# John-Jumper/Upside-MD

Measured on AMD Instinct MI355X. Metric: MD steps/sec (force evals/sec) per 300-res protein, higher is better.
Workload: dtype f32; 1 GPU; syn300_10A: 300-res synthetic protein, full side-chain BP, 10 A pair list (BASELINE.json configs[2]); 4096 independent replicas per GPU, T=0.8, dt=0.009, Langevin thermostat every round; replicas_per_gpu=4096, n_atom=900, settle_steps=100

## Files before the change

upside-md_amd/csrc/igraph_device.h:

```cpp
#pragma once
#include "device_math.h"
#include "../../include/upside_hip_kernels.h"
#include <hip/amd_detail/amd_hip_unsafe_atomics.h>

#include "env_switch.h"

struct BX { int bx, gx, by, gy; };
#define BX_REAL (BX{(int)blockIdx.x, (int)gridDim.x, (int)blockIdx.y, (int)gridDim.y})

namespace up {

__device__ __forceinline__ void bspline_basis(float y, float b[4], float d[4]) {
    const float y2 = y * y, omy = 1.f - y, omy2 = omy * omy;
    const float s = 1.f / 6.f;
    b[0] = omy2 * (omy * s);
    b[1] = fmaf(fmaf(0.5f, y, -1.f), y2, 2.f / 3.f);
    b[2] = fmaf(fmaf(fmaf(-0.5f, y, 0.5f), y, 0.5f), y, s);
    b[3] = y2 * (y * s);
    d[0] = -0.5f * omy2;
    d[1] = y * fmaf(1.5f, y, -2.f);
    d[2] = fmaf(fmaf(-1.5f, y, 1.f), y, 0.5f);
    d[3] = 0.5f * y2;
}
template <typename P>
// ... 234 lines not shown
    if (PG_LANES == 16) v += dpp_mov<UP_DPP_ROW_MIRROR>(v);
    if (PG_LANES >= 8) v += dpp_mov<UP_DPP_HALF_MIRROR>(v);
    v += dpp_mov<UP_DPP_XOR2>(v);
    v += dpp_mov<UP_DPP_XOR1>(v);
    return v;
}

template <int IT> struct list_word { typedef unsigned short type; };
template <> struct list_word<UPK_IT_ROTAMER> { typedef int type; };
static inline bool list_words_match(const upk_igraph_t* G) { return (G->word16 != 0) == (G->itype != UPK_IT_ROTAMER); }
__device__ __forceinline__ int list_word_at(const int* lists, size_t idx, int word16) {
    return word16 ? (int)((const unsigned short*)lists)[idx] : lists[idx];
}

__device__ __forceinline__ void stage_ranges(int* lds_range, unsigned short* lds_ord, const int* __restrict__ hcnt, const int* __restrict__ hlo,
                                             const unsigned short* __restrict__ ord, int n_rows) {
    for (int t = threadIdx.x; t < n_rows; t += blockDim.x) {
        lds_range[t] = (hlo ? hlo[t] : 0) | (hcnt[t] << 16);
        lds_ord[t] = ord[t];
    }
}
#define PG_WALK_LDS_WORDS(n_rows) ((n_rows) + ((n_rows) + 1) / 2)

template <typename Op, int LANES = PG_LANES, typename W = int>
__device__ __forceinline__ void group_batch_loop(Op& op, int n_rows, const unsigned short* ord, const int* range,
                                                 const W* __restrict__ hit, int cap, int* counter, int batch_first, int batch_step) {
    const int lane = threadIdx.x & 63, gl = lane & (LANES - 1), g = lane / LANES;
    const int n_batch = (n_rows + (UP_WAVE / LANES) - 1) / (UP_WAVE / LANES);
    auto claim = [&]() { int v = 0; if (lane == 0) v = atomicAdd(counter, 1); return __builtin_amdgcn_readfirstlane(v); };
    struct Batch { int row, n_mine; const W* hrow; int w[PG_CHUNK]; bool valid; };
    auto fetch = [&](int i, Batch& B) -> bool {
        const int b = batch_first + i * batch_step;
        if (b >= n_batch) return false;
        const int ri = b * (UP_WAVE / LANES) + g;
// ... 32 lines not shown
}

static inline void pair_geometry(int n_system, int n_rows, int lanes_per_row, int rows_per_full_wg, int& wgs_per_system, int& threads) {
    static const int wgs_env = env_int("UPSIDE_HIP_IG_WGS", 256);
    const int target = wgs_env < 1 ? 256 : wgs_env;
    int bps = (target + n_system - 1) / n_system;
    const int max_bps = (n_rows + rows_per_full_wg - 1) / rows_per_full_wg;
    if (bps > max_bps) bps = max_bps;
    if (bps < 1) bps = 1;
    const int rows_per_wg = (n_rows + bps - 1) / bps;
    int t = ((rows_per_wg * lanes_per_row + 63) / 64) * 64;
    threads = t < 256 ? 256 : (t > 1024 ? 1024 : t);
    wgs_per_system = bps;
}

__device__ __forceinline__ float fast_rcp(float x) { return __builtin_amdgcn_rcpf(x); }

}
```

upside-md_amd/csrc/kernels_pair.hip:

```cpp
#include "igraph_device.h"
#include "pair2_device.h"
#include <cstring>

using namespace up;
typedef unsigned short PW;

#define ST(L) ((hipStream_t)(L)->stream)
#ifndef UPK_LAUNCH_STATUS_DEFINED
#define UPK_LAUNCH_STATUS_DEFINED
static inline int launch_status() { return (int)hipGetLastError(); }
#endif
#define C_SENS(c, s) ((c).sens + (size_t)(s) * (c).n_elem * (c).stride)

struct PairArgs {
    float* out; long out_sys_stride; int out_stride, out_comp, out_row0, out_row0_2;
    float* own_grad;
    int sens_mode; const float* sens1; const float* sens2; long sens_sys_stride; int sens_stride;
    int tab_floats;
    int atomic_sens;
};

template <int IT, int ROW_SIDE, bool GRAD, bool POLY>
__device__ __forceinline__ float pair_functor(const upk_igraph_t& G, const QuadShape& Q, const float* tab, int t1, int t2,
                                              const float* x1, const float* x2, float* d) {
// ... 137 lines not shown
        if (SIDES == 3) __syncthreads();
        if (threadIdx.x == 0) *L.counter = 0;
        stage_ranges(L.range, L.ord, G.hcnt2 + (size_t)s * G.n2, nullptr, G.ord2 + (size_t)s * G.n2, G.n2);
        __syncthreads();
        RowOp<IT, 2, MODE, POLY, LANES> op(G, L, A, s);
        group_batch_loop<RowOp<IT, 2, MODE, POLY, LANES>, LANES>(op, G.n2, L.ord, L.range, (const PW*)G.hit2 + (size_t)s * G.n2 * G.cap2, G.cap2, L.counter, B.bx, B.gx);
    }
}
template <int IT, int SIDES, int MODE, bool POLY>
__global__ void __launch_bounds__(1024) PG_KERNEL_ATTR k_pair_rows(upk_igraph_t G, PairArgs A)  {
    extern __shared__ __attribute__((aligned(16))) float lds_dyn_[];
    d_pair_rows<IT, SIDES, MODE, POLY>(G, A, BX_REAL, lds_dyn_);
}

template <int DO, typename Get>
__device__ __forceinline__ void flush_other_side(float* __restrict__ osens, const int* __restrict__ oloc, int stride, int n_other, Get get) {
    for (int i = threadIdx.x; i < n_other; i += blockDim.x) {
        float add[8];
#pragma unroll
        for (int c = 0; c < 8; ++c) add[c] = c < DO ? get(c, i) : 0.f;
        float4* row = (float4*)(osens + (size_t)oloc[i] * stride);
        float4 r0 = row[0];
        r0.x += add[0]; r0.y += add[1]; r0.z += add[2]; r0.w += add[3];
        if (DO > 4) { float4 r1 = row[1]; r1.x += add[4]; r1.y += add[5]; r1.z += add[6]; r1.w += add[7]; row[1] = r1; }
        row[0] = r0;
    }
}
template <int IT, int RS, bool POLY>
struct BackwardOp {
    static constexpr int DR = RS == 1 ? PairDims<IT>::d1 : PairDims<IT>::d2;
    static constexpr int DO = RS == 1 ? PairDims<IT>::d2 : PairDims<IT>::d1;
    const upk_igraph_t& G; const QuadShape Q; const PairLds& L; unsigned long long* oacc;
// ... 120 lines not shown
        load_row8_planes(xa, RS == 1 ? L.c2 : L.c1, (RS == 1 ? G.n2 : G.n1) + 1, jA); load_row8_planes(xb, RS == 1 ? L.c2 : L.c1, (RS == 1 ? G.n2 : G.n1) + 1, jB);
        v2 xo[6];
#pragma unroll
        for (int c = 0; c < 6; ++c) xo[c] = mk2(xa[c], xb[c]);
        const int toA = __float_as_int(xa[7]), toB = __float_as_int(xb[7]);
        const v2 v = RS == 1 ? coverage_pair2<false, POLY>(G, Q, L.tab, tr, tr, toA, toB, xr, hbr, xo, nullptr, nullptr)
                             : coverage_pair2<false, POLY>(G, Q, L.tab, toA, toB, tr, tr, xo, mk2(xa[6], xb[6]), xr, nullptr, nullptr);
        acc += mk2(liveA ? v.x : 0.f, liveB ? v.y : 0.f);
    }
    __device__ __forceinline__ void flush(int row) {
        const float t = group_sum4(acc.x + acc.y);
        if ((threadIdx.x & (P2_LANES - 1)) != 0) return;
        A.out[(size_t)s * A.out_sys_stride + (size_t)((RS == 1 ? A.out_row0 : A.out_row0_2) + row) * A.out_stride + A.out_comp] = t;
    }
};
template <int RS, bool POLY>
__device__ __forceinline__ void d_cov_rows2(const upk_igraph_t& G, const PairArgs& A, const BX B, float* lds) {
        const int s = B.by;
    const PairLds L = pair2_lds(lds, G, A.tab_floats);
    stage_table(L.tab, POLY ? G.param_poly : G.param, A.tab_floats);
    const int row_len = POLY ? G.n_poly : G.n_param;
    stage_rows_planes(L.c1, G.node1, s, G.loc1, G.n1, G.dim1, G.type1, nullptr, nullptr, 0, 0.f, __int_as_float(0), G.n_type2 * row_len);
    stage_rows_planes(L.c2, G.node2, s, G.loc2, G.n2, G.dim2, G.type2, nullptr, nullptr, 0, 0.f, __int_as_float(0), row_len);
    if (threadIdx.x == 0) *L.counter = 0;
    const int n_rows = RS == 1 ? G.n1 : G.n2, cap = RS == 1 ? G.cap1 : G.cap2;
    stage_ranges(L.range, L.ord, (RS == 1 ? G.hcnt1 : G.hcnt2) + (size_t)s * n_rows, nullptr, (RS == 1 ? G.ord1 : G.ord2) + (size_t)s * n_rows, n_rows);
    __syncthreads();
    CovRowOp2<RS, POLY> op(G, L, A, s);
    group2_batch_loop(op, n_rows, L.ord, L.range, (const PW*)(RS == 1 ? G.hit1 : G.hit2) + (size_t)s * n_rows * cap, cap, L.counter, B.bx, B.gx, RS == 1 ? G.n2 : G.n1);
}
template <int RS, bool POLY>
__global__ void __launch_bounds__(1024) PG_KERNEL_ATTR k_cov_rows2(upk_igraph_t G, PairArgs A)  {
    extern __shared__ __attribute__((aligned(16))) float lds_dyn_[];
    d_cov_rows2<RS, POLY>(G, A, BX_REAL, lds_dyn_);
}

template <int RS, bool POLY>
struct CovBackwardOp2 {
    static constexpr int DR = RS == 1 ? 7 : 6, DO = RS == 1 ? 6 : 7;
    const upk_igraph_t& G; const QuadShape Q; const PairLds& L; unsigned long long* oacc;
    const bool row_has, oth_has;
    v2 xr[6], hbr, acc[DR]; float sr; int tr;
    float* row_sens; const int* row_loc; int row_stride;
    __device__ __forceinline__ CovBackwardOp2(const upk_igraph_t& G_, const PairLds& L_, unsigned long long* oacc_, int sens_mode, int s)
        : G(G_), Q(quad_shape(G_)), L(L_), oacc(oacc_), row_has(sens_mode == 3 || sens_mode == RS), oth_has(sens_mode == 3 || sens_mode == 3 - RS) {
        const upk_coord_t& node = RS == 1 ? G.node1 : G.node2;
        row_sens = node.sens + (size_t)s * node.n_elem * node.stride; row_loc = RS == 1 ? G.loc1 : G.loc2; row_stride = node.stride;
    }
    const float* site_sens = nullptr;
    __device__ __forceinline__ void begin(int row) {
// ... 34 lines not shown
#pragma unroll
            for (int c = 0; c < DO; ++c) lds_add_fixed22_scaled(oacc + c * n_o + jB, od[c].y);
        }
    }
    __device__ __forceinline__ void flush(int row) {
        float t[DR];
#pragma unroll
        for (int c = 0; c < DR; ++c) t[c] = group_sum4(acc[c].x + acc[c].y);
        if ((threadIdx.x & (P2_LANES - 1)) != 0) return;
        float* o = row_sens + (size_t)row_loc[row] * row_stride;
#pragma unroll
        for (int c = 0; c < DR; ++c) o[c] += t[c];
    }
};
template <int RS, bool POLY>
__device__ __forceinline__ void d_cov_backward2(const upk_igraph_t& G, const PairArgs& A, const BX B, float* lds) {
        constexpr int DO = CovBackwardOp2<RS, POLY>::DO;
    const int s = B.by;
    const int n_rows = RS == 1 ? G.n1 : G.n2, n_other = RS == 1 ? G.n2 : G.n1;
    const PairLds L = pair2_lds(lds, G, A.tab_floats);
    unsigned long long* oacc = (unsigned long long*)lds + (((size_t)((float*)(L.counter + 1) - lds) + 1) >> 1);
    float* site_sens = (float*)(oacc + (size_t)n_other * DO);
    const float* S1 = A.sens1 ? A.sens1 + (size_t)s * A.sens_sys_stride : nullptr;
    const float* S2 = A.sens2 ? A.sens2 + (size_t)s * A.sens_sys_stride : nullptr;
    stage_table(L.tab, POLY ? G.param_poly : G.param, A.tab_floats);
    const int row_len = POLY ? G.n_poly : G.n_param;
    stage_rows_planes(L.c1, G.node1, s, G.loc1, G.n1, G.dim1, G.type1, nullptr, nullptr, 0, 0.f, __int_as_float(0), G.n_type2 * row_len);
    stage_rows_planes(L.c2, G.node2, s, G.loc2, G.n2, G.dim2, G.type2, nullptr, S2, A.sens_stride, 0.f, __int_as_float(0), row_len);
    if (S1) for (int t = threadIdx.x; t < G.n1; t += blockDim.x) site_sens[t] = S1[(size_t)t * A.sens_stride];
    for (int t = threadIdx.x; t < n_other * DO; t += blockDim.x) oacc[t] = 0ull;
    if (threadIdx.x == 0) *L.counter = 0;
    stage_ranges(L.range, L.ord, (RS == 1 ? G.hcnt1 : G.hcnt2) + (size_t)s * n_rows, nullptr, (RS == 1 ? G.ord1 : G.ord2) + (size_t)s * n_rows, n_rows);
    __syncthreads();
    {
        CovBackwardOp2<RS, POLY> op(G, L, oacc, A.sens_mode, s);
        op.site_sens = site_sens;
        const int cap = RS == 1 ? G.cap1 : G.cap2;
        group2_batch_loop(op, n_rows, L.ord, L.range, (const PW*)(RS == 1 ? G.hit1 : G.hit2) + (size_t)s * n_rows * cap, cap, L.counter, B.bx, B.gx, n_other);
    }
    __syncthreads();
    const upk_coord_t& onode = RS == 1 ? G.node2 : G.node1;
    const int* oloc = RS == 1 ? G.loc2 : G.loc1;
    float* osens = C_SENS(onode, s);
    unsigned long long* gacc = G.gacc ? G.gacc + (size_t)s * n_other * 8 : nullptr;
    const bool alone = B.gx == 1;
    if (alone && (onode.stride & 3) == 0) { flush_other_side<DO>(osens, oloc, onode.stride, n_other, [&](int c, int i) { return from_fixed22(oacc[c * n_other + i]); }); return; }
    for (int t = threadIdx.x; t < n_other * DO; t += blockDim.x) {
        const int i = t / DO, c = t - i * DO;
        const unsigned long long a = oacc[c * n_other + i];
        if (!a) continue;
        if (alone) osens[(size_t)oloc[i] * onode.stride + c] += from_fixed22(a);
        else atomicAdd(gacc + i * 8 + c, a);
    }
}
template <int RS, bool POLY>
__global__ void __launch_bounds__(1024) PG_KERNEL_ATTR k_cov_backward2(upk_igraph_t G, PairArgs A)  {
    extern __shared__ __attribute__((aligned(16))) float lds_dyn_[];
    d_cov_backward2<RS, POLY>(G, A, BX_REAL, lds_dyn_);
}

__device__ __forceinline__ void d_pair_backward_finish(const upk_igraph_t& G, int other_side, double unit, const BX B, float* lds_unused) {
    const int s = B.by;
    const int n_other = other_side == 1 ? G.n1 : G.n2, dim = other_side == 1 ? G.dim1 : G.dim2;
    const upk_coord_t& onode = other_side == 1 ? G.node1 : G.node2;
    const int* oloc = other_side == 1 ? G.loc1 : G.loc2;
    float* osens = C_SENS(onode, s);
    unsigned long long* gacc = G.gacc + (size_t)s * n_other * 8;
    for (int t = B.bx * blockDim.x + threadIdx.x; t < n_other * 8; t += B.gx * blockDim.x) {
        const int i = t >> 3, c = t & 7;
        if (c >= dim) continue;
        const unsigned long long a = gacc[t];
        if (a) { osens[(size_t)oloc[i] * onode.stride + c] += (float)((double)(long long)a * unit); gacc[t] = 0ull; }
    }
}
// ... 13 lines not shown
    if (mode == 0) hipLaunchKernelGGL((k_pair_rows<IT, SIDES, 0, POLY>), grid, block, lds, ST(L), *G, A);
    else if (mode == 1) hipLaunchKernelGGL((k_pair_rows<IT, SIDES, 1, POLY>), grid, block, lds, ST(L), *G, A);
    else hipLaunchKernelGGL((k_pair_rows<IT, SIDES, 2, POLY>), grid, block, lds, ST(L), *G, A);
}
template <int IT, bool POLY = false>
static void rows_launch_sides(const upk_launch_t* L, const upk_igraph_t* G, int side, int mode, dim3 grid, dim3 block, size_t lds, const PairArgs& A) {
    if (side == 1) rows_launch<IT, 1, POLY>(L, G, mode, grid, block, lds, A);
    else if (side == 2) rows_launch<IT, 2, POLY>(L, G, mode, grid, block, lds, A);
    else rows_launch<IT, 3, POLY>(L, G, mode, grid, block, lds, A);
}
static int pair_table_choice(const upk_igraph_t* G, size_t extra, int& tab_floats, size_t& lds) {
    static const bool no_poly = env_int("UPSIDE_HIP_IG_POLY", 1) == 0;
    if (!no_poly && pair_lds_bytes(G, true, tab_floats, lds) && lds + extra <= 158 * 1024) return 2;
    if (pair_lds_bytes(G, false, tab_floats, lds) && lds + extra <= 158 * 1024) return 1;
    return 0;
}

extern "C" int upk_igraph_passes_staged(const upk_launch_t* L, const upk_igraph_t* G, int row_side) {
    UPK_FLUSH(L);
    (void)L;
    if (row_side != 1 && row_side != 2) return 0;
    const int n_other = row_side == 1 ? G->n2 : G->n1;
    int tab_floats; size_t lds;
    if (!pair_table_choice(G, 0, tab_floats, lds)) return 0;
    return pair_table_choice(G, 8 + (size_t)n_other * 8 * sizeof(unsigned long long), tab_floats, lds) ? 1 : 0;
}

extern "C" int upk_igraph_rows(const upk_launch_t* L, const upk_igraph_t* G, int side, int mode, float* out, long out_sys_stride,
                               int out_stride, int out_comp, int out_row0, int out_row0_2, float* own_grad, int sens_mode,
                               const float* sens1, const float* sens2, long sens_sys_stride, int sens_stride) {
// ... 10 lines not shown
    if (!table) {
        UPK_FLUSH(L);
        int r = 0;
        for (int sd = 1; sd <= 2 && !r; ++sd) {
            if (!(side & sd)) continue;
            const int row0 = sd == 1 ? A.out_row0 : A.out_row0_2;
            if (mode == 2) r = upk_igraph_grad(L, G, sd, sens_mode, sens1, sens2, sens_sys_stride, sens_stride);
            else r = upk_igraph_rowsum(L, G, sd, out, out_sys_stride, out_stride, out_comp, row0, mode == 1 ? own_grad : nullptr);
        }
        return r;
    }
    const int n_rows = side == 1 ? G->n1 : (side == 2 ? G->n2 : (G->n1 > G->n2 ? G->n1 : G->n2));
    int bps, threads;
    if (G->itype == UPK_IT_HBOND_COVERAGE && mode == 0 && side != 3 && pair2_enabled() && lds + 64 <= 158 * 1024) {
        pair_geometry(L->n_system, n_rows, P2_LANES, 256, bps, threads);
        if (side == 2 && batch_add(L, table == 2 ? BK_COV_ROWS2_POLY : BK_COV_ROWS2, bps, L->n_system, lds + 64, G, sizeof(*G), &A, sizeof(A))) return 0;
        UPK_FLUSH(L);
        const dim3 grid2(bps, L->n_system), block2(threads);
        if (side == 1) { if (table == 2) hipLaunchKernelGGL((k_cov_rows2<1, true>), grid2, block2, lds + 64, ST(L), *G, A); else hipLaunchKernelGGL((k_cov_rows2<1, false>), grid2, block2, lds + 64, ST(L), *G, A); }
        else { if (table == 2) hipLaunchKernelGGL((k_cov_rows2<2, true>), grid2, block2, lds + 64, ST(L), *G, A); else hipLaunchKernelGGL((k_cov_rows2<2, false>), grid2, block2, lds + 64, ST(L), *G, A); }
        return launch_status();
    }
    pair_geometry(L->n_system, n_rows, PG_LANES, 128, bps, threads);
    if (G->itype == UPK_IT_PROTEIN_HBOND && bps == 1) {
        threads = 256;
    }
    {
        const int bk = (G->itype == UPK_IT_PROTEIN_HBOND && side == 3 && mode == 0) ? BK_ROWS_HB_FWD : (G->itype == UPK_IT_PROTEIN_HBOND && side == 3 && mode == 2) ? BK_ROWS_HB_BWD
                     : (G->itype == UPK_IT_ENVIRONMENT && side == 1 && mode == 0) ? BK_ROWS_ENV_FWD : 0;
        if (bk && batch_add(L, bk, bps, L->n_system, lds, G, sizeof(*G), &A, sizeof(A))) return 0;
// ... 37 lines not shown
    if (!table) {
        UPK_FLUSH(L);
        int r = upk_igraph_grad(L, G, 1, sens_mode, sens1, sens2, sens_sys_stride, sens_stride);
        if (!r) r = upk_igraph_grad(L, G, 2, sens_mode, sens1, sens2, sens_sys_stride, sens_stride);
        return r;
    }
    int bps, threads;
    if (G->itype == UPK_IT_HBOND_COVERAGE && pair2_enabled()) {
        const size_t extra = 64 + (size_t)G->n1 * sizeof(float);
        size_t lds2; int tf;
        const int table2 = pair_table_choice(G, acc_bytes + extra, tf, lds2);
        if (table2) {
            A.tab_floats = tf; lds2 += acc_bytes + extra;
            pair_geometry(L->n_system, n_rows, P2_LANES, 256, bps, threads);
            if (!G->gacc) bps = 1;
            if (row_side == 2 && batch_add(L, table2 == 2 ? BK_COV_BWD2_POLY : BK_COV_BWD2, bps, L->n_system, lds2, G, sizeof(*G), &A, sizeof(A))) {
                if (bps > 1 && !batch_add(L, BK_BWD_FINISH, (n_other * 8 + 1023) / 1024, L->n_system, 0, G, sizeof(*G), nullptr, 0, 3 - row_side, 0, 1.0 / (double)(1 << P2_FIX_BITS)))
                    return finish_alone(L, G, n_other, 3 - row_side, 1.0 / (double)(1 << P2_FIX_BITS));
                return 0;
            }
            UPK_FLUSH(L);
            const dim3 grid2(bps, L->n_system), block2(threads);
            if (row_side == 1) { if (table2 == 2) hipLaunchKernelGGL((k_cov_backward2<1, true>), grid2, block2, lds2, ST(L), *G, A); else hipLaunchKernelGGL((k_cov_backward2<1, false>), grid2, block2, lds2, ST(L), *G, A); }
            else { if (table2 == 2) hipLaunchKernelGGL((k_cov_backward2<2, true>), grid2, block2, lds2, ST(L), *G, A); else hipLaunchKernelGGL((k_cov_backward2<2, false>), grid2, block2, lds2, ST(L), *G, A); }
            if (bps > 1) hipLaunchKernelGGL(k_pair_backward_finish, dim3((n_other * 8 + 255) / 256, L->n_system), dim3(256), 0, ST(L), *G, 3 - row_side, 1.0 / (double)(1 << P2_FIX_BITS));
            return launch_status();
        }
    }
    pair_geometry(L->n_system, n_rows, PG_LANES, 128, bps, threads);
    if (!G->gacc) bps = 1;
// ... 89 lines not shown
```

upside-md_amd/csrc/pair2_device.h:

```cpp
#pragma once
#include "igraph_device.h"

namespace up {

typedef float v2 __attribute__((ext_vector_type(2)));
__device__ __forceinline__ v2 mk2(float a, float b) { v2 r; r.x = a; r.y = b; return r; }
__device__ __forceinline__ v2 bc2(float a) { v2 r; r.x = a; r.y = a; return r; }
__device__ __forceinline__ v2 fma2(v2 a, v2 b, v2 c) { return __builtin_elementwise_fma(a, b, c); }

#define P2_FIX_BITS 22
#define P2_FIX_SCALE ((float)(1 << P2_FIX_BITS))
__device__ __forceinline__ unsigned long long to_fixed22_scaled(float vs) {
    int q;
    asm("v_cvt_rpi_i32_f32 %0, %1" : "=v"(q) : "v"(vs));
    return (unsigned long long)(long long)q;
}
__device__ __forceinline__ unsigned long long to_fixed22(float v) { return to_fixed22_scaled(v * P2_FIX_SCALE); }
__device__ __forceinline__ void lds_add_fixed22_scaled(unsigned long long* p, float vs) {
    __hip_atomic_fetch_add(p, to_fixed22_scaled(vs), __ATOMIC_RELAXED, __HIP_MEMORY_SCOPE_WORKGROUP);
}
__device__ __forceinline__ unsigned long long to_fixed22_wide(float v) { return (unsigned long long)__float2ll_rn(v * P2_FIX_SCALE); }
__device__ __forceinline__ void lds_add_fixed22_wide(unsigned long long* p, float v) {
    __hip_atomic_fetch_add(p, to_fixed22_wide(v), __ATOMIC_RELAXED, __HIP_MEMORY_SCOPE_WORKGROUP);
}
__device__ __forceinline__ float from_fixed22(unsigned long long a) { return (float)((double)(long long)a * (1.0 / (double)(1 << P2_FIX_BITS))); }
__device__ __forceinline__ void lds_add_fixed22(unsigned long long* p, float v) {
    __hip_atomic_fetch_add(p, to_fixed22(v), __ATOMIC_RELAXED, __HIP_MEMORY_SCOPE_WORKGROUP);
}

__device__ __forceinline__ void stage_rows_planes(float* lds, const upk_coord_t& node, int s, const int* __restrict__ loc, int n, int dim,
                                                  const int* __restrict__ meta1, const int* __restrict__ meta0,
                                                  const float* __restrict__ sens, int sens_stride, float sentinel6, float sentinel7, int meta1_mul = 1) {
    const float* base = node.out + (size_t)s * node.n_elem * node.stride;
    const int np = n + 1;
    if ((node.stride & 3) == 0) {
        for (int i = threadIdx.x; i < np; i += blockDim.x) {
            float v[8] = {0.f, 0.f, 0.f, 0.f, 0.f, 0.f, 0.f, 0.f};
            if (i == n) { v[0] = v[1] = v[2] = 1.0e4f; v[3] = 1.f; v[6] = sentinel6; v[7] = sentinel7; }
            else {
                const int l = loc[i];
                const int m1 = meta1 ? meta1[i] * meta1_mul : 0, m0 = meta0 ? meta0[i] : 0;
                const float sv = sens ? sens[(size_t)i * sens_stride] : 0.f;
                const float4* row = (const float4*)(base + (size_t)l * node.stride);
                const float4 r0 = row[0];
                float4 r1 = make_float4(0.f, 0.f, 0.f, 0.f);
                if (dim > 4) r1 = row[1];
                const float r[8] = {r0.x, r0.y, r0.z, r0.w, r1.x, r1.y, r1.z, r1.w};
#pragma unroll
                for (int c = 0; c < 8; ++c) v[c] = c < dim ? r[c] : 0.f;
                if (dim <= 7 && meta1) v[7] = __int_as_float(m1);
                if (dim <= 6) { if (sens) v[6] = sv; else if (meta0) v[6] = __int_as_float(m0); }
            }
            ((float4*)lds)[i] = make_float4(v[0], v[1], v[2], v[3]);
            ((float4*)lds)[np + i] = make_float4(v[4], v[5], v[6], v[7]);
        }
        return;
    }
    for (int t = threadIdx.x; t < np * 8; t += blockDim.x) {
        const int i = t >> 3, c = t & 7;
        float v = 0.f;
        if (i == n) v = c < 3 ? 1.0e4f : (c == 3 ? 1.f : (c == 6 ? sentinel6 : (c == 7 ? sentinel7 : 0.f)));
        else if (c < dim) v = base[(size_t)loc[i] * node.stride + c];
        else if (c == 7 && meta1) v = __int_as_float(meta1[i] * meta1_mul);
        else if (c == 6 && sens) v = sens[(size_t)i * sens_stride];
        else if (c == 6 && meta0) v = __int_as_float(meta0[i]);
        lds[(c >> 2) * np * 4 + i * 4 + (c & 3)] = v;
    }
}
__device__ __forceinline__ void load_row8_planes(float* x, const float* planes, int np, int j) {
    const float4 lo = *(const float4*)(planes + j * 4), hi = *(const float4*)(planes + (np + j) * 4);
    x[0] = lo.x; x[1] = lo.y; x[2] = lo.z; x[3] = lo.w; x[4] = hi.x; x[5] = hi.y; x[6] = hi.z; x[7] = hi.w;
}

__device__ __forceinline__ void cubic2(const float* cA, const float* cB, v2 y, v2& v, v2& d) {
    const float4 a = *(const float4*)cA, b = *(const float4*)cB;
    const v2 c0 = mk2(a.x, b.x), c1 = mk2(a.y, b.y), c2 = mk2(a.z, b.z), c3 = mk2(a.w, b.w);
    const v2 t = fma2(c3, y, c2), s = fma2(t, y, c1);
    v = fma2(s, y, c0);
    d = fma2(fma2(c3, y, t), y, s);
}
__device__ __forceinline__ v2 cubic2_value(const float* cA, const float* cB, v2 y) {
// ... 172 lines not shown
```

Before: 222,800 system-steps/s.

## Add persistent resident coverage-pair kernels that prefetch the next system into registers

Adds persistent kernels for the hbond-coverage pair forward and backward passes. Each workgroup loops over systems with a grid-stride step, keeps the parameter table resident in LDS, and loads the next system's node planes, sensitivities and row ranges into registers before the barrier, then writes them to LDS. The backward variant re-zeroes its accumulators while flushing, which avoids a separate zeroing pass. Resident mode is taken by default when there are at least twice as many systems as CUs, with the grid sized from an occupancy query. This saves per-workgroup launch and table-staging cost but adds register pressure and forces one workgroup per system. Optional phase-clock instrumentation is included.

After: 222,400 system-steps/s. About the same (-0.2%).

```diff
diff --git a/upside-md_amd/csrc/igraph_device.h b/upside-md_amd/csrc/igraph_device.h
--- a/upside-md_amd/csrc/igraph_device.h
+++ b/upside-md_amd/csrc/igraph_device.h
@@ -272,10 +272,28 @@
 }
 
 __device__ __forceinline__ void stage_ranges(int* lds_range, unsigned short* lds_ord, const int* __restrict__ hcnt, const int* __restrict__ hlo,
-                                             const unsigned short* __restrict__ ord, int n_rows) {
-    for (int t = threadIdx.x; t < n_rows; t += blockDim.x) {
+                                             const unsigned short* __restrict__ ord, int n_rows, int t0 = threadIdx.x) {
+    for (int t = t0; t < n_rows; t += blockDim.x) {
         lds_range[t] = (hlo ? hlo[t] : 0) | (hcnt[t] << 16);
         lds_ord[t] = ord[t];
+    }
+}
+#ifndef PG_PF_TRIPS
+#define PG_PF_TRIPS 2
+#endif
+struct RangeRegs { int range[PG_PF_TRIPS]; unsigned short ord[PG_PF_TRIPS]; };
+__device__ __forceinline__ void load_ranges_regs(RangeRegs& r, int t0, const int* __restrict__ hcnt, const unsigned short* __restrict__ ord, int n_rows) {
+#pragma unroll
+    for (int u = 0; u < PG_PF_TRIPS; ++u) {
+        const int t = t0 + u * blockDim.x;
+        if (t < n_rows) { r.range[u] = hcnt[t] << 16; r.ord[u] = ord[t]; }
+    }
+}
+__device__ __forceinline__ void stage_ranges_regs(int* lds_range, unsigned short* lds_ord, const RangeRegs& r, int n_rows, int t0) {
+#pragma unroll
+    for (int u = 0; u < PG_PF_TRIPS; ++u) {
+        const int t = t0 + u * blockDim.x;
+        if (t < n_rows) { lds_range[t] = r.range[u]; lds_ord[t] = r.ord[u]; }
     }
 }
 #define PG_WALK_LDS_WORDS(n_rows) ((n_rows) + ((n_rows) + 1) / 2)
@@ -338,6 +356,37 @@
     wgs_per_system = bps;
 }
 
+static inline int pair_persist_mode() {
+    static const int mode = env_set("UPSIDE_HIP_PAIR_PERSIST") ? (env_int("UPSIDE_HIP_PAIR_PERSIST", 0) != 0 ? 1 : 0) : -1;
+    return mode;
+}
+static inline void pair_persist_force_geometry(int& wgs_per_system, int& threads) {
+    if (pair_persist_mode() == 1 && wgs_per_system > 1) { wgs_per_system = 1; threads = 1024; }
+}
+template <auto KERNEL>
+static inline int pair_resident_grid(int n_system, int wgs_per_system, int threads, size_t lds) {
+    const int mode = pair_persist_mode();
+    static const int wgs_env = env_int("UPSIDE_HIP_PAIR_PERSIST_WGS", 0);
+    if (mode == 0 || wgs_per_system != 1 || n_system < 1) return 0;
+    if (mode < 0 && n_system < 2 * upk_device_cu_count()) return 0;
+    if (wgs_env > 0) return wgs_env;
+    static int per_cu = 0, per_cu_threads = 0; static size_t per_cu_lds = 0;
+    if (!per_cu || per_cu_threads != threads || per_cu_lds != lds) {
+        int n = 0;
+        if (hipOccupancyMaxActiveBlocksPerMultiprocessor(&n, (const void*)KERNEL, threads, lds) != hipSuccess || n < 1) { (void)hipGetLastError(); n = 1; }
+        per_cu = n; per_cu_threads = threads; per_cu_lds = lds;
+    }
+    const long g = (long)per_cu * upk_device_cu_count();
+    return (int)(g < n_system ? g : n_system);
+}
+
+template <typename T> __device__ __forceinline__ const T& kernarg_fresh() {
+    auto p = __builtin_amdgcn_kernarg_segment_ptr();
+    asm volatile("" : "+s"(p));
+    return *(const T*)p;
+}
+__device__ __forceinline__ int lane_fresh() { int t = threadIdx.x; asm volatile("" : "+v"(t)); return t; }
+
 __device__ __forceinline__ float fast_rcp(float x) { return __builtin_amdgcn_rcpf(x); }
 
 }
diff --git a/upside-md_amd/csrc/kernels_pair.hip b/upside-md_amd/csrc/kernels_pair.hip
--- a/upside-md_amd/csrc/kernels_pair.hip
+++ b/upside-md_amd/csrc/kernels_pair.hip
@@ -175,8 +175,8 @@
 }
 
 template <int DO, typename Get>
-__device__ __forceinline__ void flush_other_side(float* __restrict__ osens, const int* __restrict__ oloc, int stride, int n_other, Get get) {
-    for (int i = threadIdx.x; i < n_other; i += blockDim.x) {
+__device__ __forceinline__ void flush_other_side(float* __restrict__ osens, const int* __restrict__ oloc, int stride, int n_other, Get get, int t0 = threadIdx.x) {
+    for (int i = t0; i < n_other; i += blockDim.x) {
         float add[8];
 #pragma unroll
         for (int c = 0; c < 8; ++c) add[c] = c < DO ? get(c, i) : 0.f;
@@ -327,26 +327,131 @@
         A.out[(size_t)s * A.out_sys_stride + (size_t)((RS == 1 ? A.out_row0 : A.out_row0_2) + row) * A.out_stride + A.out_comp] = t;
     }
 };
+#ifdef UPK_PHASE_CLOCKS
+#define PHASE_RECORDS 16384
+__device__ unsigned long long g_phase[2 * PHASE_RECORDS * 8];
+struct PhaseClock {
+    unsigned long long* r;
+    __device__ __forceinline__ PhaseClock(int bwd, int n1, int s, int served, unsigned long long wg_start)
+        : r(g_phase + ((size_t)bwd * PHASE_RECORDS + (s < PHASE_RECORDS ? s : 0)) * 8) {
+        if (threadIdx.x == 0) {
+            const unsigned hw = __builtin_amdgcn_s_getreg((31 << 11) | 4), xcc = __builtin_amdgcn_s_getreg((31 << 11) | 20);
+            r[2] = ~0ull; r[5] = ((unsigned long long)(xcc & 0xf) << 16) | (hw & 0xff00); r[6] = wg_start + 1; r[7] = (unsigned long long)served | ((unsigned long long)n1 << 32);
+        }
+    }
+    __device__ __forceinline__ void at(int slot) const { if (threadIdx.x == 0) r[slot] = wall_clock64(); }
+    __device__ __forceinline__ void first_out() const { if ((threadIdx.x & 63) == 0) atomicMin(r + 2, (unsigned long long)wall_clock64()); }
+};
+extern "C" int upk_phase_clocks_read(unsigned long long* out, int n_records) {
+    if (n_records > 2 * PHASE_RECORDS) n_records = 2 * PHASE_RECORDS;
+    return (int)hipMemcpyFromSymbol(out, HIP_SYMBOL(g_phase), (size_t)n_records * 8 * sizeof(unsigned long long));
+}
+#define PHASE(x) x
+#else
+#define PHASE(x)
+#endif
+
+template <int RS, bool POLY, bool BWD>
+struct Cov2Stage {
+    struct Regs { PlanesRegs e1, e2; RangeRegs rr; float ss[P2_PF_TRIPS]; };
+    const upk_igraph_t& G; const PairArgs& A; const PairLds& L; float* site_sens; const int row_len, n_rows;
+    __device__ __forceinline__ Cov2Stage(const upk_igraph_t& G_, const PairArgs& A_, const PairLds& L_, float* site_sens_)
+        : G(G_), A(A_), L(L_), site_sens(site_sens_), row_len(POLY ? G_.n_poly : G_.n_param), n_rows(RS == 1 ? G_.n1 : G_.n2) {}
+    __device__ __forceinline__ const float* S1(int s) const { return BWD && A.sens1 ? A.sens1 + (size_t)s * A.sens_sys_stride : nullptr; }
+    __device__ __forceinline__ const float* S2(int s) const { return BWD && A.sens2 ? A.sens2 + (size_t)s * A.sens_sys_stride : nullptr; }
+    __device__ __forceinline__ const int* hcnt(int s) const { return (RS == 1 ? G.hcnt1 : G.hcnt2) + (size_t)s * n_rows; }
+    __device__ __forceinline__ const unsigned short* ord(int s) const { return (RS == 1 ? G.ord1 : G.ord2) + (size_t)s * n_rows; }
+    __device__ __forceinline__ void direct(int s, int t0 = threadIdx.x) const {
+        stage_rows_planes(L.c1, G.node1, s, G.loc1, G.n1, G.dim1, G.type1, nullptr, nullptr, 0, 0.f, __int_as_float(0), G.n_type2 * row_len, t0);
+        stage_rows_planes(L.c2, G.node2, s, G.loc2, G.n2, G.dim2, G.type2, nullptr, S2(s), A.sens_stride, 0.f, __int_as_float(0), row_len, t0);
+        if (BWD) { const float* s1 = S1(s); if (s1) for (int t = t0; t < G.n1; t += blockDim.x) site_sens[t] = s1[(size_t)t * A.sens_stride]; }
+        if (threadIdx.x == 0) *L.counter = 0;
+        stage_ranges(L.range, L.ord, hcnt(s), nullptr, ord(s), n_rows, t0);
+    }
+    __device__ __forceinline__ void load(int s, Regs& r) const {
+        const int t0 = lane_fresh();
+        load_planes_regs(r.e1, t0, G.node1, s, G.loc1, G.n1, G.dim1, G.type1, nullptr, nullptr, 0, 0.f, __int_as_float(0), G.n_type2 * row_len);
+        load_planes_regs(r.e2, t0, G.node2, s, G.loc2, G.n2, G.dim2, G.type2, nullptr, S2(s), A.sens_stride, 0.f, __int_as_float(0), row_len);
+        if (BWD) {
+            const float* s1 = S1(s);
+#pragma unroll
+            for (int u = 0; u < P2_PF_TRIPS; ++u) { const int t = t0 + u * blockDim.x; r.ss[u] = s1 && t < G.n1 ? s1[(size_t)t * A.sens_stride] : 0.f; }
+        }
+        load_ranges_regs(r.rr, t0, hcnt(s), ord(s), n_rows);
+    }
+    __device__ __forceinline__ void store(int s, const Regs& r) const {
+        const int t0 = lane_fresh();
+        stage_planes_regs(L.c1, r.e1, G.n1, t0);
+        stage_planes_regs(L.c2, r.e2, G.n2, t0);
+        if (BWD && A.sens1) {
+#pragma unroll
+            for (int u = 0; u < P2_PF_TRIPS; ++u) { const int t = t0 + u * blockDim.x; if (t < G.n1) site_sens[t] = r.ss[u]; }
+        }
+        stage_ranges_regs(L.range, L.ord, r.rr, n_rows, t0);
+        const int held = P2_PF_TRIPS * blockDim.x;
+        if (G.n1 + 1 > held || G.n2 + 1 > held || n_rows > held) direct(s, t0 + held);
+        else if (threadIdx.x == 0) *L.counter = 0;
+    }
+};
+static_assert(P2_PF_TRIPS == PG_PF_TRIPS, "Cov2Stage::store takes one count of register-held trips for elements and rows");
+
+template <int RS, bool POLY>
+__device__ __forceinline__ void cov_rows2_loop(const upk_igraph_t& G, const PairArgs& A, const PairLds& L, int s, int bx, int gx) {
+    const int n_rows = RS == 1 ? G.n1 : G.n2, cap = RS == 1 ? G.cap1 : G.cap2;
+    CovRowOp2<RS, POLY> op(G, L, A, s);
+    group2_batch_loop(op, n_rows, L.ord, L.range, (const PW*)(RS == 1 ? G.hit1 : G.hit2) + (size_t)s * n_rows * cap, cap, L.counter, bx, gx, RS == 1 ? G.n2 : G.n1);
+}
 template <int RS, bool POLY>
 __device__ __forceinline__ void d_cov_rows2(const upk_igraph_t& G, const PairArgs& A, const BX B, float* lds) {
-        const int s = B.by;
+    const int s = B.by;
     const PairLds L = pair2_lds(lds, G, A.tab_floats);
     stage_table(L.tab, POLY ? G.param_poly : G.param, A.tab_floats);
-    const int row_len = POLY ? G.n_poly : G.n_param;
-    stage_rows_planes(L.c1, G.node1, s, G.loc1, G.n1, G.dim1, G.type1, nullptr, nullptr, 0, 0.f, __int_as_float(0), G.n_type2 * row_len);
-    stage_rows_planes(L.c2, G.node2, s, G.loc2, G.n2, G.dim2, G.type2, nullptr, nullptr, 0, 0.f, __int_as_float(0), row_len);
-    if (threadIdx.x == 0) *L.counter = 0;
-    const int n_rows = RS == 1 ? G.n1 : G.n2, cap = RS == 1 ? G.cap1 : G.cap2;
-    stage_ranges(L.range, L.ord, (RS == 1 ? G.hcnt1 : G.hcnt2) + (size_t)s * n_rows, nullptr, (RS == 1 ? G.ord1 : G.ord2) + (size_t)s * n_rows, n_rows);
+    PHASE(const unsigned long long t_start = wall_clock64(); const PhaseClock clk(0, G.n1, s, 0, t_start); if (threadIdx.x == 0) clk.r[0] = t_start;)
+    Cov2Stage<RS, POLY, false>(G, A, L, nullptr).direct(s);
     __syncthreads();
-    CovRowOp2<RS, POLY> op(G, L, A, s);
-    group2_batch_loop(op, n_rows, L.ord, L.range, (const PW*)(RS == 1 ? G.hit1 : G.hit2) + (size_t)s * n_rows * cap, cap, L.counter, B.bx, B.gx, RS == 1 ? G.n2 : G.n1);
+    PHASE(clk.at(1);)
+    cov_rows2_loop<RS, POLY>(G, A, L, s, B.bx, B.gx);
+    PHASE(clk.first_out(); __syncthreads(); clk.at(3); clk.at(4);)
 }
 template <int RS, bool POLY>
 __global__ void __launch_bounds__(1024) PG_KERNEL_ATTR k_cov_rows2(upk_igraph_t G, PairArgs A)  {
     extern __shared__ __attribute__((aligned(16))) float lds_dyn_[];
     d_cov_rows2<RS, POLY>(G, A, BX_REAL, lds_dyn_);
 }
+struct Cov2ResidentArgs { upk_igraph_t G; PairArgs A; int n_system; };
+#define COV2_PHASE_FWD const Cov2ResidentArgs& K = kernarg_fresh<Cov2ResidentArgs>(); const PairLds L = pair2_lds(lds_dyn_, K.G, K.A.tab_floats); \
+                       const Cov2Stage<RS, POLY, false> stage(K.G, K.A, L, nullptr)
+template <int RS, bool POLY>
+__global__ void __launch_bounds__(1024) PG_KERNEL_ATTR k_cov_rows2_resident(Cov2ResidentArgs)  {
+    extern __shared__ __attribute__((aligned(16))) float lds_dyn_[];
+    int s = blockIdx.x;
+    PHASE(const unsigned long long t_start = wall_clock64(); unsigned long long t_turn = t_start; int served = 0;)
+    {
+        COV2_PHASE_FWD;
+        if (s >= K.n_system) return;
+        stage_table(L.tab, POLY ? K.G.param_poly : K.G.param, K.A.tab_floats);
+        stage.direct(s);
+    }
+    for (;;) {
+        PHASE(const PhaseClock clk(0, kernarg_fresh<Cov2ResidentArgs>().G.n1, s, served++, t_start); if (threadIdx.x == 0) clk.r[0] = t_turn;)
+        __syncthreads();
+        PHASE(clk.at(1);)
+        { COV2_PHASE_FWD; cov_rows2_loop<RS, POLY>(K.G, K.A, L, s, 0, 1); }
+        PHASE(clk.first_out();)
+        const int next = s + gridDim.x;
+        typename Cov2Stage<RS, POLY, false>::Regs r = {};
+        {
+            COV2_PHASE_FWD;
+            if (next >= K.n_system) { PHASE(__syncthreads(); clk.at(3); clk.at(4);) break; }
+            stage.load(next, r);
+        }
+        __syncthreads();
+        PHASE(clk.at(3); clk.at(4); t_turn = wall_clock64();)
+        { COV2_PHASE_FWD; stage.store(next, r); }
+        s = next;
+    }
+}
+#undef COV2_PHASE_FWD
 
 template <int RS, bool POLY>
 struct CovBackwardOp2 {
@@ -411,50 +516,107 @@
     }
 };
 template <int RS, bool POLY>
-__device__ __forceinline__ void d_cov_backward2(const upk_igraph_t& G, const PairArgs& A, const BX B, float* lds) {
-        constexpr int DO = CovBackwardOp2<RS, POLY>::DO;
-    const int s = B.by;
-    const int n_rows = RS == 1 ? G.n1 : G.n2, n_other = RS == 1 ? G.n2 : G.n1;
-    const PairLds L = pair2_lds(lds, G, A.tab_floats);
-    unsigned long long* oacc = (unsigned long long*)lds + (((size_t)((float*)(L.counter + 1) - lds) + 1) >> 1);
-    float* site_sens = (float*)(oacc + (size_t)n_other * DO);
-    const float* S1 = A.sens1 ? A.sens1 + (size_t)s * A.sens_sys_stride : nullptr;
-    const float* S2 = A.sens2 ? A.sens2 + (size_t)s * A.sens_sys_stride : nullptr;
-    stage_table(L.tab, POLY ? G.param_poly : G.param, A.tab_floats);
-    const int row_len = POLY ? G.n_poly : G.n_param;
-    stage_rows_planes(L.c1, G.node1, s, G.loc1, G.n1, G.dim1, G.type1, nullptr, nullptr, 0, 0.f, __int_as_float(0), G.n_type2 * row_len);
-    stage_rows_planes(L.c2, G.node2, s, G.loc2, G.n2, G.dim2, G.type2, nullptr, S2, A.sens_stride, 0.f, __int_as_float(0), row_len);
-    if (S1) for (int t = threadIdx.x; t < G.n1; t += blockDim.x) site_sens[t] = S1[(size_t)t * A.sens_stride];
-    for (int t = threadIdx.x; t < n_other * DO; t += blockDim.x) oacc[t] = 0ull;
-    if (threadIdx.x == 0) *L.counter = 0;
-    stage_ranges(L.range, L.ord, (RS == 1 ? G.hcnt1 : G.hcnt2) + (size_t)s * n_rows, nullptr, (RS == 1 ? G.ord1 : G.ord2) + (size_t)s * n_rows, n_rows);
-    __syncthreads();
-    {
-        CovBackwardOp2<RS, POLY> op(G, L, oacc, A.sens_mode, s);
-        op.site_sens = site_sens;
-        const int cap = RS == 1 ? G.cap1 : G.cap2;
-        group2_batch_loop(op, n_rows, L.ord, L.range, (const PW*)(RS == 1 ? G.hit1 : G.hit2) + (size_t)s * n_rows * cap, cap, L.counter, B.bx, B.gx, n_other);
-    }
-    __syncthreads();
+struct CovBwd2Lds {
+    static constexpr int DO = CovBackwardOp2<RS, POLY>::DO;
+    unsigned long long* oacc; float* site_sens; int n_other;
+    __device__ __forceinline__ CovBwd2Lds(const upk_igraph_t& G, const PairLds& L, float* lds) {
+        n_other = RS == 1 ? G.n2 : G.n1;
+        oacc = (unsigned long long*)lds + (((size_t)((float*)(L.counter + 1) - lds) + 1) >> 1);
+        site_sens = (float*)(oacc + (size_t)n_other * DO);
+    }
+    __device__ __forceinline__ void zero() const { for (int t = threadIdx.x; t < n_other * DO; t += blockDim.x) oacc[t] = 0ull; }
+};
+template <int RS, bool POLY>
+__device__ __forceinline__ void cov_backward2_loop(const upk_igraph_t& G, const PairArgs& A, const PairLds& L, const CovBwd2Lds<RS, POLY>& W, int s, int bx, int gx) {
+    const int n_rows = RS == 1 ? G.n1 : G.n2, cap = RS == 1 ? G.cap1 : G.cap2;
+    CovBackwardOp2<RS, POLY> op(G, L, W.oacc, A.sens_mode, s);
+    op.site_sens = W.site_sens;
+    group2_batch_loop(op, n_rows, L.ord, L.range, (const PW*)(RS == 1 ? G.hit1 : G.hit2) + (size_t)s * n_rows * cap, cap, L.counter, bx, gx, W.n_other);
+}
+template <int RS, bool POLY, bool REARM>
+__device__ __forceinline__ void cov_backward2_hand_over(const upk_igraph_t& G, const CovBwd2Lds<RS, POLY>& W, int s, int gx) {
+    constexpr int DO = CovBwd2Lds<RS, POLY>::DO;
+    const int n_other = W.n_other;
+    unsigned long long* oacc = W.oacc;
     const upk_coord_t& onode = RS == 1 ? G.node2 : G.node1;
     const int* oloc = RS == 1 ? G.loc2 : G.loc1;
     float* osens = C_SENS(onode, s);
     unsigned long long* gacc = G.gacc ? G.gacc + (size_t)s * n_other * 8 : nullptr;
-    const bool alone = B.gx == 1;
-    if (alone && (onode.stride & 3) == 0) { flush_other_side<DO>(osens, oloc, onode.stride, n_other, [&](int c, int i) { return from_fixed22(oacc[c * n_other + i]); }); return; }
+    const bool alone = gx == 1;
+    if (alone && (onode.stride & 3) == 0) {
+        flush_other_side<DO>(osens, oloc, onode.stride, n_other, [&](int c, int i) {
+            const unsigned long long a = oacc[c * n_other + i];
+            if (REARM) oacc[c * n_other + i] = 0ull;
+            return from_fixed22(a);
+        }, REARM ? lane_fresh() : (int)threadIdx.x);
+        return;
+    }
     for (int t = threadIdx.x; t < n_other * DO; t += blockDim.x) {
         const int i = t / DO, c = t - i * DO;
         const unsigned long long a = oacc[c * n_other + i];
         if (!a) continue;
+        if (REARM) oacc[c * n_other + i] = 0ull;
         if (alone) osens[(size_t)oloc[i] * onode.stride + c] += from_fixed22(a);
         else atomicAdd(gacc + i * 8 + c, a);
     }
+}
+template <int RS, bool POLY>
+__device__ __forceinline__ void d_cov_backward2(const upk_igraph_t& G, const PairArgs& A, const BX B, float* lds) {
+    const int s = B.by;
+    const PairLds L = pair2_lds(lds, G, A.tab_floats);
+    const CovBwd2Lds<RS, POLY> W(G, L, lds);
+    stage_table(L.tab, POLY ? G.param_poly : G.param, A.tab_floats);
+    PHASE(const unsigned long long t_start = wall_clock64(); const PhaseClock clk(1, G.n1, s, 0, t_start); if (threadIdx.x == 0) clk.r[0] = t_start;)
+    Cov2Stage<RS, POLY, true>(G, A, L, W.site_sens).direct(s);
+    W.zero();
+    __syncthreads();
+    PHASE(clk.at(1);)
+    cov_backward2_loop<RS, POLY>(G, A, L, W, s, B.bx, B.gx);
+    PHASE(clk.first_out();)
+    __syncthreads();
+    PHASE(clk.at(3);)
+    cov_backward2_hand_over<RS, POLY, false>(G, W, s, B.gx);
+    PHASE(__syncthreads(); clk.at(4);)
 }
 template <int RS, bool POLY>
 __global__ void __launch_bounds__(1024) PG_KERNEL_ATTR k_cov_backward2(upk_igraph_t G, PairArgs A)  {
     extern __shared__ __attribute__((aligned(16))) float lds_dyn_[];
     d_cov_backward2<RS, POLY>(G, A, BX_REAL, lds_dyn_);
 }
+#define COV2_PHASE_BWD const Cov2ResidentArgs& K = kernarg_fresh<Cov2ResidentArgs>(); const PairLds L = pair2_lds(lds_dyn_, K.G, K.A.tab_floats); \
+                       const CovBwd2Lds<RS, POLY> W(K.G, L, lds_dyn_); const Cov2Stage<RS, POLY, true> stage(K.G, K.A, L, W.site_sens)
+template <int RS, bool POLY>
+__global__ void __launch_bounds__(1024) PG_KERNEL_ATTR k_cov_backward2_resident(Cov2ResidentArgs)  {
+    extern __shared__ __attribute__((aligned(16))) float lds_dyn_[];
+    int s = blockIdx.x;
+    PHASE(const unsigned long long t_start = wall_clock64(); unsigned long long t_turn = t_start; int served = 0;)
+    {
+        COV2_PHASE_BWD;
+        if (s >= K.n_system) return;
+        stage_table(L.tab, POLY ? K.G.param_poly : K.G.param, K.A.tab_floats);
+        stage.direct(s);
+        W.zero();
+    }
+    for (;;) {
+        PHASE(const PhaseClock clk(1, kernarg_fresh<Cov2ResidentArgs>().G.n1, s, served++, t_start); if (threadIdx.x == 0) clk.r[0] = t_turn;)
+        __syncthreads();
+        PHASE(clk.at(1);)
+        { COV2_PHASE_BWD; (void)stage; cov_backward2_loop<RS, POLY>(K.G, K.A, L, W, s, 0, 1); }
+        PHASE(clk.first_out();)
+        const int next = s + gridDim.x;
+        bool more;
+        typename Cov2Stage<RS, POLY, true>::Regs r = {};
+        { COV2_PHASE_BWD; more = next < K.n_system; if (more) stage.load(next, r); }
+        __syncthreads();
+        PHASE(clk.at(3); t_turn = wall_clock64();)
+        { COV2_PHASE_BWD; (void)stage; cov_backward2_hand_over<RS, POLY, true>(K.G, W, s, 1); }
+        PHASE(clk.at(4);)
+        if (!more) break;
+        { COV2_PHASE_BWD; stage.store(next, r); }
+        s = next;
+    }
+}
+#undef COV2_PHASE_BWD
 
 __device__ __forceinline__ void d_pair_backward_finish(const upk_igraph_t& G, int other_side, double unit, const BX B, float* lds_unused) {
     const int s = B.by;
@@ -498,6 +660,25 @@
     if (!no_poly && pair_lds_bytes(G, true, tab_floats, lds) && lds + extra <= 158 * 1024) return 2;
     if (pair_lds_bytes(G, false, tab_floats, lds) && lds + extra <= 158 * 1024) return 1;
     return 0;
+}
+
+#define COV2_RESIDENT_INSTANCES(X) \
+    if (!bwd && rs == 1 && poly) { X((k_cov_rows2_resident<1, true>)); } else if (!bwd && rs == 1) { X((k_cov_rows2_resident<1, false>)); } \
+    else if (!bwd && poly) { X((k_cov_rows2_resident<2, true>)); } else if (!bwd) { X((k_cov_rows2_resident<2, false>)); } \
+    else if (rs == 1) { X((k_cov_backward2_resident<1, true>)); } else { X((k_cov_backward2_resident<2, true>)); }
+static int cov2_resident_grid(const upk_launch_t* L, const upk_igraph_t* G, bool bwd, int rs, bool poly, int& bps, int& threads, size_t lds) {
+    if ((G->node1.stride & 3) || (G->node2.stride & 3)) return 0;
+    if (bwd && !poly) return 0;
+    pair_persist_force_geometry(bps, threads);
+#define X(K) return pair_resident_grid<&K>(L->n_system, bps, threads, lds)
+    COV2_RESIDENT_INSTANCES(X)
+#undef X
+}
+static void cov2_resident_launch(const upk_launch_t* L, const upk_igraph_t* G, const PairArgs& A, bool bwd, int rs, bool poly, int grid, int threads, size_t lds) {
+    Cov2ResidentArgs K; K.G = *G; K.A = A; K.n_system = L->n_system;
+#define X(KERNEL) hipLaunchKernelGGL(KERNEL, dim3(grid), dim3(threads), lds, ST(L), K)
+    COV2_RESIDENT_INSTANCES(X)
+#undef X
 }
 
 extern "C" int upk_igraph_passes_staged(const upk_launch_t* L, const upk_igraph_t* G, int row_side) {
@@ -538,6 +719,11 @@
     int bps, threads;
     if (G->itype == UPK_IT_HBOND_COVERAGE && mode == 0 && side != 3 && pair2_enabled() && lds + 64 <= 158 * 1024) {
         pair_geometry(L->n_system, n_rows, P2_LANES, 256, bps, threads);
+        if (const int rg = cov2_resident_grid(L, G, false, side, table == 2, bps, threads, lds + 64)) {
+            UPK_FLUSH(L);
+            cov2_resident_launch(L, G, A, false, side, table == 2, rg, threads, lds + 64);
+            return launch_status();
+        }
         if (side == 2 && batch_add(L, table == 2 ? BK_COV_ROWS2_POLY : BK_COV_ROWS2, bps, L->n_system, lds + 64, G, sizeof(*G), &A, sizeof(A))) return 0;
         UPK_FLUSH(L);
         const dim3 grid2(bps, L->n_system), block2(threads);
@@ -605,6 +791,11 @@
             A.tab_floats = tf; lds2 += acc_bytes + extra;
             pair_geometry(L->n_system, n_rows, P2_LANES, 256, bps, threads);
             if (!G->gacc) bps = 1;
+            if (const int rg = cov2_resident_grid(L, G, true, row_side, table2 == 2, bps, threads, lds2)) {
+                UPK_FLUSH(L);
+                cov2_resident_launch(L, G, A, true, row_side, table2 == 2, rg, threads, lds2);
+                return launch_status();
+            }
             if (row_side == 2 && batch_add(L, table2 == 2 ? BK_COV_BWD2_POLY : BK_COV_BWD2, bps, L->n_system, lds2, G, sizeof(*G), &A, sizeof(A))) {
                 if (bps > 1 && !batch_add(L, BK_BWD_FINISH, (n_other * 8 + 1023) / 1024, L->n_system, 0, G, sizeof(*G), nullptr, 0, 3 - row_side, 0, 1.0 / (double)(1 << P2_FIX_BITS)))
                     return finish_alone(L, G, n_other, 3 - row_side, 1.0 / (double)(1 << P2_FIX_BITS));
diff --git a/upside-md_amd/csrc/pair2_device.h b/upside-md_amd/csrc/pair2_device.h
--- a/upside-md_amd/csrc/pair2_device.h
+++ b/upside-md_amd/csrc/pair2_device.h
@@ -28,35 +28,43 @@
     __hip_atomic_fetch_add(p, to_fixed22(v), __ATOMIC_RELAXED, __HIP_MEMORY_SCOPE_WORKGROUP);
 }
 
+__device__ __forceinline__ void planes_elem(float4& lo, float4& hi, const float* base, int stride, const int* __restrict__ loc, int n, int dim,
+                                            const int* __restrict__ meta1, const int* __restrict__ meta0, const float* __restrict__ sens, int sens_stride,
+                                            float sentinel6, float sentinel7, int meta1_mul, int i) {
+    float v[8] = {0.f, 0.f, 0.f, 0.f, 0.f, 0.f, 0.f, 0.f};
+    if (i == n) { v[0] = v[1] = v[2] = 1.0e4f; v[3] = 1.f; v[6] = sentinel6; v[7] = sentinel7; }
+    else {
+        const int l = loc[i];
+        const int m1 = meta1 ? meta1[i] * meta1_mul : 0, m0 = meta0 ? meta0[i] : 0;
+        const float sv = sens ? sens[(size_t)i * sens_stride] : 0.f;
+        const float4* row = (const float4*)(base + (size_t)l * stride);
+        const float4 r0 = row[0];
+        float4 r1 = make_float4(0.f, 0.f, 0.f, 0.f);
+        if (dim > 4) r1 = row[1];
+        const float r[8] = {r0.x, r0.y, r0.z, r0.w, r1.x, r1.y, r1.z, r1.w};
+#pragma unroll
+        for (int c = 0; c < 8; ++c) v[c] = c < dim ? r[c] : 0.f;
+        if (dim <= 7 && meta1) v[7] = __int_as_float(m1);
+        if (dim <= 6) { if (sens) v[6] = sv; else if (meta0) v[6] = __int_as_float(m0); }
+    }
+    lo = make_float4(v[0], v[1], v[2], v[3]);
+    hi = make_float4(v[4], v[5], v[6], v[7]);
+}
 __device__ __forceinline__ void stage_rows_planes(float* lds, const upk_coord_t& node, int s, const int* __restrict__ loc, int n, int dim,
                                                   const int* __restrict__ meta1, const int* __restrict__ meta0,
-                                                  const float* __restrict__ sens, int sens_stride, float sentinel6, float sentinel7, int meta1_mul = 1) {
+                                                  const float* __restrict__ sens, int sens_stride, float sentinel6, float sentinel7, int meta1_mul = 1, int t0 = threadIdx.x) {
     const float* base = node.out + (size_t)s * node.n_elem * node.stride;
     const int np = n + 1;
     if ((node.stride & 3) == 0) {
-        for (int i = threadIdx.x; i < np; i += blockDim.x) {
-            float v[8] = {0.f, 0.f, 0.f, 0.f, 0.f, 0.f, 0.f, 0.f};
-            if (i == n) { v[0] = v[1] = v[2] = 1.0e4f; v[3] = 1.f; v[6] = sentinel6; v[7] = sentinel7; }
-            else {
-                const int l = loc[i];
-                const int m1 = meta1 ? meta1[i] * meta1_mul : 0, m0 = meta0 ? meta0[i] : 0;
-                const float sv = sens ? sens[(size_t)i * sens_stride] : 0.f;
-                const float4* row = (const float4*)(base + (size_t)l * node.stride);
-                const float4 r0 = row[0];
-                float4 r1 = make_float4(0.f, 0.f, 0.f, 0.f);
-                if (dim > 4) r1 = row[1];
-                const float r[8] = {r0.x, r0.y, r0.z, r0.w, r1.x, r1.y, r1.z, r1.w};
-#pragma unroll
-                for (int c = 0; c < 8; ++c) v[c] = c < dim ? r[c] : 0.f;
-                if (dim <= 7 && meta1) v[7] = __int_as_float(m1);
-                if (dim <= 6) { if (sens) v[6] = sv; else if (meta0) v[6] = __int_as_float(m0); }
-            }
-            ((float4*)lds)[i] = make_float4(v[0], v[1], v[2], v[3]);
-            ((float4*)lds)[np + i] = make_float4(v[4], v[5], v[6], v[7]);
+        for (int i = t0; i < np; i += blockDim.x) {
+            float4 lo, hi;
+            planes_elem(lo, hi, base, node.stride, loc, n, dim, meta1, meta0, sens, sens_stride, sentinel6, sentinel7, meta1_mul, i);
+            ((float4*)lds)[i] = lo;
+            ((float4*)lds)[np + i] = hi;
         }
         return;
     }
-    for (int t = threadIdx.x; t < np * 8; t += blockDim.x) {
+    for (int t = (t0 - (int)threadIdx.x) * 8 + threadIdx.x; t < np * 8; t += blockDim.x) {
         const int i = t >> 3, c = t & 7;
         float v = 0.f;
         if (i == n) v = c < 3 ? 1.0e4f : (c == 3 ? 1.f : (c == 6 ? sentinel6 : (c == 7 ? sentinel7 : 0.f)));
@@ -65,6 +73,28 @@
         else if (c == 6 && sens) v = sens[(size_t)i * sens_stride];
         else if (c == 6 && meta0) v = __int_as_float(meta0[i]);
         lds[(c >> 2) * np * 4 + i * 4 + (c & 3)] = v;
+    }
+}
+#ifndef P2_PF_TRIPS
+#define P2_PF_TRIPS 2
+#endif
+struct PlanesRegs { float4 lo[P2_PF_TRIPS], hi[P2_PF_TRIPS]; };
+__device__ __forceinline__ void load_planes_regs(PlanesRegs& r, int t0, const upk_coord_t& node, int s, const int* __restrict__ loc, int n, int dim,
+                                                 const int* __restrict__ meta1, const int* __restrict__ meta0,
+                                                 const float* __restrict__ sens, int sens_stride, float sentinel6, float sentinel7, int meta1_mul = 1) {
+    const float* base = node.out + (size_t)s * node.n_elem * node.stride;
+#pragma unroll
+    for (int u = 0; u < P2_PF_TRIPS; ++u) {
+        const int i = t0 + u * blockDim.x;
+        if (i <= n) planes_elem(r.lo[u], r.hi[u], base, node.stride, loc, n, dim, meta1, meta0, sens, sens_stride, sentinel6, sentinel7, meta1_mul, i);
+    }
+}
+__device__ __forceinline__ void stage_planes_regs(float* lds, const PlanesRegs& r, int n, int t0) {
+    const int np = n + 1;
+#pragma unroll
+    for (int u = 0; u < P2_PF_TRIPS; ++u) {
+        const int i = t0 + u * blockDim.x;
+        if (i < np) { ((float4*)lds)[i] = r.lo[u]; ((float4*)lds)[np + i] = r.hi[u]; }
     }
 }
 __device__ __forceinline__ void load_row8_planes(float* x, const float* planes, int np, int j) {
```
